# KirillKryukov/naf

Hardware: AMD Instinct MI355X
Metric: unnaf GB/s (uncompressed bases out) on 100 GB synthetic FASTA (higher is better)
Workload: dtype u8; 1 GPU; unnaf decode of a 100.0 GB synthetic-ACGT FASTA archive on one GPU (the size BASELINE.json's metric is quoted on; configs[1] at 10 GB rides along as cfg10_*), 100 records, 80-col lines; archive made in-run by the GPU ennaf; .naf 24739662224 B -> FASTA 99999995684 B, text + archive + decoded text resident in HBM; parallelism=one archive, one GPU, no data-path collective

## Files before the change

naf_amd/csrc/emit.hip:

```cpp
#include "ctx.h"
#include "wgscan.h"
#include "emit_core.h"
#include "packed.h"
#include <thread>

__device__ __forceinline__ void st_text16(u8 *p, const uint4 &v, int nt)
{
    if (nt) {
        u32x4 nv; nv.x = v.x; nv.y = v.y; nv.z = v.z; nv.w = v.w;
        __builtin_nontemporal_store(nv, (u32x4 *)p);
    } else *(uint4 *)p = v;
}

__global__ void k_len_flags(const u32 *units, u64 n, u64 *flag)
{
    u64 i = (u64)blockIdx.x * blockDim.x + threadIdx.x;
    if (i < n) flag[i] = units[i] != 0xFFFFFFFFu;
}
__global__ void k_len_acc(const u32 *units, u64 n, const u64 *ridx, u64 *rec_len, u64 N)
{
    u64 i = (u64)blockIdx.x * blockDim.x + threadIdx.x;
    if (i < n && ridx[i] < N) atomicAdd((unsigned long long *)&rec_len[ridx[i]], (unsigned long long)units[i]);
}

// ... 109 lines not shown
            if (v != 255) {
                if ((u64)nt + size > cap) { ok = false; break; }
                for (u32 k = t; k < size; k += 256) toggles[nt + k] = base + (u64)v * (k + 1);
                nt += size;
            }
            base += (u64)v * size; units += size; pos += 4;
        } else if (type == 0) {
            if ((u64)pos + 3 + size > len) { ok = false; break; }
            const u8 *rb = mbuf + pos + 3;
            const u32 per = (size + 255) / 256, lo = t * per < size ? t * per : size, hi = lo + per < size ? lo + per : size;
            u64 sm = 0, cn = 0;
            for (u32 k = lo; k < hi; k++) { const u32 u = rb[k]; sm += u; cn += u != 255; }
            u64 tot_s, tot_c;
            const u64 is = wg_scan_inclusive<u64, OpAdd>(sm, &tot_s, lds);
            const u64 ic = wg_scan_inclusive<u64, OpAdd>(cn, &tot_c, lds);
            if (nt + tot_c > cap) { ok = false; break; }
            u64 at = base + is - sm; u32 idx = nt + (u32)(ic - cn);
            for (u32 k = lo; k < hi; k++) { const u32 u = rb[k]; at += u; if (u != 255) toggles[idx++] = at; }
            base += tot_s; nt += (u32)tot_c; units += size; pos += 3 + size;
        } else ok = false;
        if (last) done = true;
    }
    ok = ok && done && pos == len && units == expect_units;
    if (t == 0) { res[0] = ok ? 1 : 0; res[1] = nt; res[2] = units; }
}

__device__ __forceinline__ void rec_size_of(u64 r, u64 len, const u64 *idz, const u64 *nmz, int has_ids, int has_names, int mode, u64 L, u32 *hdr, u64 *out)
{
    u64 h = 0;
    if (mode == EM_FASTA || mode == EM_FASTQ) {
        u64 idl = 0, nml = 0;
        if (has_ids) idl = idz[r] - (r ? idz[r - 1] + 1 : 0);
        if (has_names) nml = nmz[r] - (r ? nmz[r - 1] + 1 : 0);
        u64 name = has_ids ? idl + ((has_names && nml) ? 1 + nml : 0) : nml;
        h = 1 + name + 1;
    }
    u64 body;
    if (mode == EM_FASTQ) body = 2 * len + 4;
    else if (mode == EM_SEQUENCES) body = len + 1;
    else body = len ? len + (L ? (len + L - 1) / L : 1) : 0;
    *hdr = (u32)h; *out = h + body;
}
__global__ void k_rec_sizes(u64 N, const u64 *rec_len, const u64 *idz, const u64 *nmz, int has_ids, int has_names,
                            int mode, u64 L, u32 *hdr_len, u64 *out_size, u64 *base_size)
{
    u64 r = (u64)blockIdx.x * blockDim.x + threadIdx.x;
    if (r >= N) return;
// ... 535 lines not shown
        }
        if (g == 0) { os[len] = '\n'; os[len + 1] = '+'; os[len + 2] = '\n'; os[2 * len + 3] = '\n'; }
        group_copy<ER_LANES>(os + len + 3, P.qual + base, len, g);
    }
    if (!in_lds) return;
    __syncthreads();
    u8 *dst = out + wbase; const u32 n = (u32)wspan;
    u32 head = (u32)((16 - ((uintptr_t)dst & 15)) & 15); if (head > n) head = n;
    if (threadIdx.x < head) dst[threadIdx.x] = stage[threadIdx.x];
    u32 words = (n - head) >> 4;
    for (u32 w = threadIdx.x; w < words; w += WGT) {
        u64 a, b2; __builtin_memcpy(&a, stage + head + 16 * w, 8); __builtin_memcpy(&b2, stage + head + 16 * w + 8, 8);
        uint4 v; v.x = (u32)a; v.y = (u32)(a >> 32); v.z = (u32)b2; v.w = (u32)(b2 >> 32);
        st_text16(dst + head + 16 * w, v, P.nt_store);
    }
    for (u32 k = head + 16 * words + threadIdx.x; k < n; k += WGT) dst[k] = stage[k];
}

#define EMIT_TOG_LDS 256u
struct TileIdx { u64 gline, k, khi; u32 col, fast; };
#define TI_HDR 0xFFFFFFFFu
struct TileFlat { u64 q0, A, q1, A1, q2, qf; };
struct TileFlatE { u64 base, a1_addr; u32 a1_sh, K0, K1, d1, d2, qoff, par0, pad; };
static_assert(sizeof(TileFlatE) == sizeof(TileFlat), "the derived record replaces the raw one in place");
#define FLAT_QM 4096
#define TILE_WG 255
__global__ __launch_bounds__(256) void k_tile_index(EmitP P, u64 ntiles, TileIdx *ti, u64 *tr, u32 *list, u32 *count, TileFlat *tsig, u32 spare, u32 *list2)
{
    __shared__ u64 s_k[256], s_r[256];
    const u64 t = (u64)blockIdx.x * TILE_WG + threadIdx.x;
    const u64 p = P.out_begin + t * 4096;
    TileIdx x; x.fast = 0; x.gline = 0; x.khi = 0; x.k = P.n_toggles; x.col = TI_HDR;
    TileFlat f; f.q0 = f.A = f.q1 = f.A1 = f.q2 = f.qf = 0;
    u64 r = ~0ull; u32 cbits = 1;
    const bool inside = t < ntiles && p < P.out_end;
    if (inside) {
        u64 g;
        if (P.mode == EM_SEQ) { r = 0; x.col = 0; g = p; x.gline = p; }
        else {
            r = upper_bound_u64(P.rec_out, 0, P.N + 1, p) - 1;
            u64 off = p - P.rec_out[r], hl = P.hdr_len[r], len = P.rec_len[r], j = 0;
            if (off >= hl) {
                u64 q = off - hl;
                if (P.mode == EM_FASTA && P.L) {
                    u64 line = q / (P.L + 1), col = q - line * (P.L + 1);
                    j = line * P.L + (col < P.L ? col : P.L);
                    if (P.L < 0xFFFFFFF0ull) { x.gline = P.rec_base[r] + line * P.L; x.col = (u32)col; }
                } else if (P.mode != EM_FASTQ) { j = q; x.col = 0; x.gline = P.rec_base[r] + q; }
                if (j > len) j = len;
            }
            g = P.rec_base[r] + j;
        }
        x.k = P.masking ? upper_bound_u64(P.toggles, 0, P.n_toggles, g) : 0;
// ... 2 lines not shown
            const u64 q = g >> 1;
            u64 lo, hi, gs = q >> 13; if (gs >= P.fslots) gs = P.fslots - 1;
            if (si[gs].q0 <= q) { lo = gs; hi = gs + 1; u64 st = 1; while (hi < P.fslots && si[hi].q0 <= q) { lo = hi; st <<= 1; hi = lo + st; } if (hi > P.fslots) hi = P.fslots; }
            else { hi = gs; u64 st = 1; lo = gs - 1; while (lo > 0 && si[lo].q0 > q) { hi = lo; st <<= 1; lo = lo > st ? lo - st : 0; } }
            while (hi - lo > 1) { const u64 mid = (lo + hi) >> 1; if (si[mid].q0 <= q) lo = mid; else hi = mid; }
            f.q0 = si[lo].q0; f.A = si[lo].A; f.qf = q;
            if (P.fcls) {
                u32 c = 3; u64 b = lo >> 2; const u64 nb = P.fslots >> 2, qe = q + 2048 + 16;
                for (u32 k = 0; k < 6 && b < nb && si[4 * b].q0 <= qe; k++, b++) c &= P.fcls[b];
                if (b < nb && si[4 * b].q0 <= qe) c = 0;
                cbits = c;
            }
            u64 cs = lo + 1;
            while (cs < P.fslots && si[cs + 1].q0 == si[cs].q0) cs++;
            f.q1 = si[cs].q0; f.A1 = cs < P.fslots ? si[cs].A : 0;
            u64 ce = cs < P.fslots ? cs + 1 : cs;
            while (ce < P.fslots && si[ce + 1].q0 == si[ce].q0) ce++;
            f.q2 = si[ce].q0;
        }
    }
    s_k[threadIdx.x] = x.k; s_r[threadIdx.x] = r;
    __syncthreads();
    if (threadIdx.x == TILE_WG) return;
    TileFlatE e; e.base = (u64)P.fsrc; e.a1_addr = (u64)P.fsrc; e.a1_sh = 4; e.K0 = e.K1 = 0; e.d1 = e.d2 = 0x7FFFFFFFu; e.qoff = 0; e.par0 = 0; e.pad = 0;
    if (t >= ntiles) {
        if (t == ntiles) { tr[t] = ~0ull; ti[t] = x; if (tsig && spare) *(TileFlatE *)&tsig[t] = e; }
        else if (tsig && t < ntiles + spare) { ti[t].fast = 0; *(TileFlatE *)&tsig[t] = e; }
        return;
    }
    tr[t] = r;
    if (!inside) { ti[t] = x; if (tsig) *(TileFlatE *)&tsig[t] = e; list[atomicAdd(count, 1u)] = (u32)t; return; }
    const u64 r_next = s_r[threadIdx.x + 1];
    x.khi = s_k[threadIdx.x + 1];
    const bool wrap = P.mode == EM_FASTA && P.L != 0;
    bool fast = x.col != TI_HDR && r == r_next && P.out_begin + (t + 1) * 4096 <= P.out_end && !P.force_slow && (!wrap || P.L >= 16);
    bool packed = false;
    if (tsig) {
        packed = fast && (cbits & 2);
        if (fast && !(cbits & 1)) fast = false;
        if (fast) {
            fast = f.qf + 2048 + 16 < f.q2 || f.q2 == f.q1;
            if (P.ftail && f.qf + 2048 + 16 >= P.ftail_q) fast = false;
            if (f.q2 != f.q1 && (f.A1 > f.A ? f.A1 - f.A : f.A - f.A1) >= (1ull << 29)) fast = false;
        }
        if (fast) {
            const u64 gline = x.gline;
            const u64 dd1 = f.q1 - f.qf, dd2 = f.q2 - f.qf;
            e.d1 = dd1 > 0x7FFFFFFFull ? 0x7FFFFFFFu : (u32)dd1; e.d2 = dd2 > 0x7FFFFFFFull ? 0x7FFFFFFFu : (u32)dd2;
            const u64 T0 = f.A - 4 * (f.qf - f.q0), T1 = f.A1 + 4 * (u64)e.d1;
            const bool two = f.q2 != f.q1;
            const u64 tmin = two && T1 < T0 ? T1 : T0;
            const u64 ub = (tmin - 40 - 4 * (u64)FLAT_QM) & ~7ull;
            e.base = (u64)P.fsrc + (u64)((i64)ub >> 3);
            e.K0 = (u32)(T0 - 40 - ub); e.K1 = two ? (u32)(T1 - 40 - ub) : e.K0;
            e.qoff = (u32)((gline >> 1) - f.qf); e.par0 = (u32)gline & 1u;
            const u64 t1 = (f.A1 < 40 ? 40 : f.A1) - 40;
            e.a1_addr = (u64)P.fsrc + (t1 >> 3); e.a1_sh = (u32)(t1 & 7) + 4;
        }
        *(TileFlatE *)&tsig[t] = e;
    }
    x.fast = fast ? 1u : (packed ? 2u : 0u);
    ti[t] = x;
    if (!fast) { if (packed) list2[atomicAdd(count + 1, 1u)] = (u32)t; else list[atomicAdd(count, 1u)] = (u32)t; }
}

template <bool FOURBIT>
__device__ __forceinline__ void emit_tile_body(const EmitP &P, const TileIdx &a, u8 *out_tile)
{
    __shared__ u64 s_tog[EMIT_TOG_LDS];
    const u32 ntog = (u32)(a.khi - a.k < EMIT_TOG_LDS ? a.khi - a.k : EMIT_TOG_LDS);
    const bool use_tog = P.masking && a.k < a.khi && a.khi - a.k <= EMIT_TOG_LDS;
    if (use_tog) { for (u32 i = threadIdx.x; i < ntog; i += 256) s_tog[i] = P.toggles[a.k + i]; __syncthreads(); }
    const u32 lane16 = threadIdx.x * 16;
    u64 g0; u32 nl_b = 64;
    if (P.mode == EM_FASTA && P.L != 0) {
        const u32 Lp1 = (u32)P.L + 1;
        u32 c = a.col + lane16, dl;
        if (Lp1 < 32768) dl = __umulhi(c, P.Ldiv_magic); else dl = c >= Lp1 ? 1u : 0u;
        u32 col = c - dl * Lp1;
        g0 = a.gline + (u64)dl * (u32)P.L + col;
        u32 d = (u32)P.L - col;
        nl_b = d < 16 ? d : 64;
    } else g0 = a.gline + lane16;
    u64 lo, hi;
    if (FOURBIT) {
// ... 228 lines not shown
            u32 w0 = s_pair[h >> 24], w1 = s_pair[(h >> 16) & 0xFFu], w2 = s_pair[(h >> 8) & 0xFFu], w3 = s_pair[h & 0xFFu];
            if (g0 & 1) {
                const u32 c9 = s_pair[n9 << 4];
                w0 = __builtin_amdgcn_alignbyte(w1, w0, 1); w1 = __builtin_amdgcn_alignbyte(w2, w1, 1);
                w2 = __builtin_amdgcn_alignbyte(w3, w2, 1); w3 = __builtin_amdgcn_alignbyte(c9, w3, 1);
            }
            lo = (u64)w0 | ((u64)w1 << 32); hi = (u64)w2 | ((u64)w3 << 32);
        }
        const u32 ntog = (u32)(a.khi - a.k < EMIT_TOG_LDS ? a.khi - a.k : EMIT_TOG_LDS);
        const bool use_tog = P.masking && a.k < a.khi && a.khi - a.k <= EMIT_TOG_LDS;
        if (use_tog) mask16_from(s_tog[j], ntog, a.k, g0, lo, hi);
        else mask16(P, a.k, a.khi, P.masking && a.k < a.khi, g0, lo, hi);
        uint4 v; v.x = (u32)lo; v.y = (u32)(lo >> 32); v.z = (u32)hi; v.w = (u32)(hi >> 32);
        if (nls[j] < 16) {
            const uint4 sel = s_spl[2 * nls[j]], orv = s_spl[2 * nls[j] + 1];
            const u32 x0 = v.x, x1 = v.y, x2 = v.z, x3 = v.w;
            v.x = __builtin_amdgcn_perm(x0, 0u, sel.x) | orv.x; v.y = __builtin_amdgcn_perm(x1, x0, sel.y) | orv.y;
            v.z = __builtin_amdgcn_perm(x2, x1, sel.z) | orv.z; v.w = __builtin_amdgcn_perm(x3, x2, sel.w) | orv.w;
        }
        st_text16(out + t * 4096 + lane16, v, P.nt_store);
    }
}

template <u32 TW>
__global__ __launch_bounds__(64) void k_emit_tile_flat_wave(EmitP P, const TileIdx *ti, const TileFlat *tsig, u8 *out, u64 ntiles, u32 xcd_chunk)
{
    u32 wg = blockIdx.x;
    if (xcd_chunk) { wg = (blockIdx.x & 7u) * xcd_chunk + (blockIdx.x >> 3); if ((u64)wg * TW >= ntiles) return; }
    __shared__ u64 s_tog[TW][EMIT_TOG_LDS];
    __shared__ uint4 s_spl[32];
    __shared__ u32 s_pair[256];
    const u32 lane = threadIdx.x;
    if (lane < 32) s_spl[lane] = ((const uint4 *)(P.fpair + 272))[lane];
    ((uint4 *)s_pair)[lane] = ((const uint4 *)(P.fpair + 16))[lane];
    TileIdx A[TW]; TileFlatE F[TW]; bool live[TW];
    {
        const u64 t0 = (u64)wg * TW;
        const uint4 *pa = (const uint4 *)(ti + t0), *pf = (const uint4 *)(tsig + t0);
        uint4 ra[2 * TW], rf[3 * TW];
#pragma unroll
        for (u32 i = 0; i < 2 * TW; i++) ra[i] = pa[i];
#pragma unroll
        for (u32 i = 0; i < 3 * TW; i++) rf[i] = pf[i];
#pragma unroll
        for (u32 j = 0; j < TW; j++) {
            __builtin_memcpy(&A[j], &ra[2 * j], 32); __builtin_memcpy(&F[j], &rf[3 * j], 48);
            live[j] = t0 + j < ntiles && A[j].fast == 1;
        }
    }
    u64 X[TW][4]; u32 grels[TW][4], pk[TW][4];
#pragma unroll
    for (u32 j = 0; j < TW; j++) {
        const TileIdx &a = A[j]; const TileFlatE &e = F[j];
#pragma unroll
        for (u32 r = 0; r < 4; r++) {
            const u32 lane16 = (r * 64 + lane) * 16;
            u32 grel, nl_b = 64;
            if (P.mode == EM_FASTA && P.L != 0) {
                const u32 Lp1 = (u32)P.L + 1;
                u32 c = a.col + lane16, dl;
                if (Lp1 < 32768) dl = __umulhi(c, P.Ldiv_magic); else dl = c >= Lp1 ? 1u : 0u;
                u32 col = c - dl * Lp1;
                grel = dl * (u32)P.L + col;
                u32 d = (u32)P.L - col;
                nl_b = d < 16 ? d : 64;
            } else grel = lane16;
            grels[j][r] = grel;
            const u32 par = e.par0 + grel;
            const u32 need = 8 + (par & 1u);
            const u32 qrel = (par >> 1) + e.qoff;
            const bool second = qrel >= e.d1;
            const u32 qm = live[j] ? ~0u : 0u;
            const u32 off = (second ? e.K1 : e.K0) - ((4 * qrel) & qm);
            const u32 rem = (second ? e.d2 : e.d1) - qrel;
            X[j][r] = ldg_at_unaligned<u64>(e.base + (off >> 3));
            pk[j][r] = nl_b | ((need > rem ? rem : 16u) << 8) | ((off & 7u) << 16);
        }
    }
    if (P.masking) {
#pragma unroll
        for (u32 j = 0; j < TW; j++) {
            const u64 nt = A[j].khi - A[j].k;
            for (u32 i = lane; i < EMIT_TOG_LDS; i += 64) s_tog[j][i] = (live[j] && i < nt && nt <= EMIT_TOG_LDS) ? P.toggles[A[j].k + i] : 0ull;
        }
    }
    __syncthreads();
#pragma unroll
    for (u32 j = 0; j < TW; j++) {
        const u64 t = (u64)wg * TW + j;
        if (!live[j]) continue;
        const TileIdx &a = A[j];
        const u32 ntog = (u32)(a.khi - a.k < EMIT_TOG_LDS ? a.khi - a.k : EMIT_TOG_LDS);
        const bool use_tog = P.masking && a.k < a.khi && a.khi - a.k <= EMIT_TOG_LDS;
#pragma unroll
        for (u32 r = 0; r < 4; r++) {
            const u64 g0 = a.gline + grels[j][r];
            const u32 nl = pk[j][r] & 0xFFu, have = (pk[j][r] >> 8) & 0xFFu;
            u64 h36 = X[j][r] >> ((pk[j][r] >> 16) + 4);
            if (have < 9) {
                const u64 y = ldg_at_unaligned<u64>(F[j].a1_addr);
                const u64 n36 = (y >> F[j].a1_sh) & 0xFFFFFFFFFull;
                const u32 keep = 4 * have;
                h36 = (h36 & ~(0xFFFFFFFFFull >> keep)) | (n36 >> keep);
            }
            const u32 h = (u32)(h36 >> 4), n9 = (u32)h36 & 15u;
            u64 lo, hi;
            {
                u32 w0 = s_pair[h >> 24], w1 = s_pair[(h >> 16) & 0xFFu], w2 = s_pair[(h >> 8) & 0xFFu], w3 = s_pair[h & 0xFFu];
                if (g0 & 1) {
                    const u32 c9 = s_pair[n9 << 4];
                    w0 = __builtin_amdgcn_alignbyte(w1, w0, 1); w1 = __builtin_amdgcn_alignbyte(w2, w1, 1);
                    w2 = __builtin_amdgcn_alignbyte(w3, w2, 1); w3 = __builtin_amdgcn_alignbyte(c9, w3, 1);
                }
                lo = (u64)w0 | ((u64)w1 << 32); hi = (u64)w2 | ((u64)w3 << 32);
            }
            if (use_tog) mask16_from(s_tog[j], ntog, a.k, g0, lo, hi);
            else mask16(P, a.k, a.khi, P.masking && a.k < a.khi, g0, lo, hi);
            uint4 v; v.x = (u32)lo; v.y = (u32)(lo >> 32); v.z = (u32)hi; v.w = (u32)(hi >> 32);
            if (nl < 16) {
                const uint4 sel = s_spl[2 * nl], orv = s_spl[2 * nl + 1];
                const u32 x0 = v.x, x1 = v.y, x2 = v.z, x3 = v.w;
                v.x = __builtin_amdgcn_perm(x0, 0u, sel.x) | orv.x; v.y = __builtin_amdgcn_perm(x1, x0, sel.y) | orv.y;
                v.z = __builtin_amdgcn_perm(x2, x1, sel.z) | orv.z; v.w = __builtin_amdgcn_perm(x3, x2, sel.w) | orv.w;
            }
            st_text16(out + t * 4096 + (r * 64 + lane) * 16, v, P.nt_store);
        }
    }
}

template <bool FOURBIT>
__device__ __forceinline__ void emit_rest_tile(const EmitP &P, const TileIdx *ti, const u64 *tr, u64 t, u8 *out, u32 chunk)
{
    const TileIdx a = ti[t];
    u64 p0 = P.out_begin + t * 4096 + chunk * 16;
    if (p0 >= P.out_end) return;
    u32 nbytes = P.out_end - p0 < 16 ? (u32)(P.out_end - p0) : 16;
    const u32 Lp1_32 = (P.L + 1) >> 32 ? 0 : (u32)(P.L + 1);
    u8 *o = out + (p0 - P.out_begin);
    if (P.mode == EM_SEQ) {
        for (u32 bb = 0; bb < nbytes; bb++) o[bb] = (u8)emit_byte<FOURBIT>(P, p0 + bb, 0, 0, a.k, a.khi);
// ... 169 lines not shown
{
    ContainerOut *d_co = arena_new<ContainerOut>(c, 1); if (!d_co) return NAF_GPU_ENOMEM;
    LAUNCH(c, "unnaf_parse_container", k_parse_container, 1, 64, 0, (const u8 *)d_naf, (u64)len, d_co);
    int rc = ctx_readback(c, co, d_co, sizeof *co); if (rc) return rc;
    if (co->code) { char buf[160]; container_error_text(co->code, &co->h, buf, sizeof buf); return ctx_fail(c, NAF_GPU_EFORMAT, "%s", buf); }
    return 0;
}

extern "C" int naf_gpu_parse_header(naf_gpu_ctx *c, const void *d_naf, size_t len, naf_gpu_header *h)
{
    if (!c || !h) return NAF_GPU_EARG;
    arena_reset(c);
    ContainerOut co;
    int rc = parse_container_device(c, d_naf, len, &co);
    *h = co.h;
    return rc;
}

enum { S_IDS = 0, S_NAMES, S_LEN, S_MASK, S_SEQ, S_QUAL };

struct UnnafPlan {
    naf_gpu_header h; u8 frame_head[6][24]; EmitP P; u64 total; bool fourbit; bool empty;
    u64 seq_bytes; bool need_qual;
    u64 main_total, surplus, sur_c, sur_base0;
};

static int load_section(naf_gpu_ctx *c, const u8 *d_naf, const naf_gpu_header &h, int i, u64 expect, const char *what, u8 **out, const u8 *head = nullptr)
{
    u8 *buf = (u8 *)arena_alloc(c, expect + 32);
    if (!buf) return NAF_GPU_ENOMEM;
    size_t n = 0;
    int rc = zstd_decode(c, d_naf + h.payload_off[i], h.comp_size[i], 0, buf, expect, &n, head);
    if (rc == NAF_GPU_ECAP || (rc == 0 && n != expect)) return ctx_fail(c, NAF_GPU_EFORMAT, "can't decompress %s\n", what);
    if (rc) return rc;
    *out = buf;
    return 0;
}

static int unnaf_prepare(naf_gpu_ctx *c, const u8 *d_naf, size_t naf_len, const naf_gpu_unnaf_opts *o, UnnafPlan &pl)
{
    ContainerOut co;
    int rc = parse_container_device(c, d_naf, naf_len, &co); if (rc) return rc;
    pl.h = co.h; memcpy(pl.frame_head, co.frame_head, sizeof pl.frame_head);
    const naf_gpu_header &h = pl.h;
    EmitP &P = pl.P; memset(&P, 0, sizeof P);
    int has_mask = (h.flags >> 2) & 1, has_data = (h.flags >> 1) & 1, has_qual = h.flags & 1;
// ... 93 lines not shown
    HIP_TRY(x, hipMemsetAsync(rec_len, 0, (N + 1) * 8, x->stream));
    if (n_len) LAUNCH(x, "unnaf_len_flags", k_len_flags, cdiv(n_len, 256), 256, 0, (const u32 *)lens, n_len, flag);
    if ((r = scan_exclusive_u64(x, flag, n_len, flag + n_len + 1))) return r;
    if (n_len) LAUNCH(x, "unnaf_len_acc", k_len_acc, cdiv(n_len, 256), 256, 0, (const u32 *)lens, n_len, (const u64 *)flag, rec_len, N);
    u64 nrec = 0;
    if ((r = ctx_readback(x, &nrec, flag + n_len + 1, 8))) return r;
    if (nrec < N) return ctx_fail(x, NAF_GPU_EFORMAT, "corrupted lengths: %llu records described, %llu expected", (unsigned long long)nrec, (unsigned long long)N);
    return 0;
}

static int mask_rle_frame(naf_gpu_ctx *x, SideCall &S, bool *done)
{
    const naf_gpu_header &h = S.h; EmitP &P = S.P;
    const u64 cs = h.comp_size[S_MASK], n_mask = h.orig_size[S_MASK];
    *done = false;
    if (!(cs >= 4 && cs <= MASK_RLE_SRC && n_mask >= 2 * cs) || ctx_opt_is(x, "MASK_RLE", '0')) return 0;
    const u8 fhd = S.pl.frame_head[S_MASK][0];
    const u32 fcs_flag = fhd >> 6, single = (fhd >> 5) & 1;
    const u32 hdr_size = 1 + (single ? 0 : 1) + (fcs_flag == 0 ? single : (fcs_flag == 1 ? 2 : (fcs_flag == 2 ? 4 : 8)));
    if ((fhd & 0x0F) || hdr_size >= cs) return 0;
    u64 *tg = arena_new<u64>(x, MASK_RLE_TOG + 1), *d_res = arena_new<u64>(x, 4);
    if (!tg || !d_res) return NAF_GPU_ENOMEM;
    LAUNCH(x, "unnaf_mask_rle", k_mask_rle_frame, 1, 256, (u32)((cs + 15) & ~15ull), S.d_naf + h.payload_off[S_MASK], (u32)cs, hdr_size, n_mask, tg, MASK_RLE_TOG, d_res);
    u64 res[3] = { 0, 0, 0 };
    int r = ctx_readback(x, res, d_res, 24); if (r) return r;
    if (res[0] == 1) { P.toggles = tg; P.n_toggles = res[1]; *done = true; }
    return 0;
}

static int mask_toggles(naf_gpu_ctx *x, SideCall &S)
{
    const naf_gpu_header &h = S.h; EmitP &P = S.P;
    int r; bool done;
    u8 *mu = nullptr; const u64 n_mask = h.orig_size[S_MASK];
    if ((r = mask_rle_frame(x, S, &done)) || done) return r;
    if ((r = load_section(x, S.d_naf, h, S_MASK, n_mask, "mask", &mu, S.pl.frame_head[S_MASK]))) return r;
    u64 tiles = (n_mask + MT_TILE - 1) / MT_TILE;
    u64 *ts = arena_new<u64>(x, tiles + 2), *tc = arena_new<u64>(x, tiles + 2);
    if (!ts || !tc) return NAF_GPU_ENOMEM;
    if (tiles) LAUNCH(x, "unnaf_mask_count", k_mask_count, tiles, 256, 0, (const u8 *)mu, n_mask, ts, tc);
    if ((r = scan_exclusive_u64(x, ts, tiles, (u64 *)nullptr))) return r;
    if ((r = scan_exclusive_u64(x, tc, tiles, tc + tiles + 1))) return r;
    u64 ntog = 0;
    if ((r = ctx_readback(x, &ntog, tc + tiles + 1, 8))) return r;
    u64 *tg = arena_new<u64>(x, ntog + 1);
    if (!tg) return NAF_GPU_ENOMEM;
    if (tiles) LAUNCH(x, "unnaf_mask_scatter", k_mask_scatter, tiles, 256, 0, (const u8 *)mu, n_mask, (const u64 *)ts, (const u64 *)tc, tg, ntog);
    P.toggles = tg; P.n_toggles = ntog;
    return 0;
}

static void side_mask_meanwhile(naf_gpu_ctx *c, SideCall &S)
{
    if (!S.mask_meanwhile) return;
    S.mask_ran = true; S.rc_mask = mask_toggles(c, S);
    if (S.rc_mask) memcpy(S.mask_err, c->err, sizeof c->err);
}

static int side_fused_launch(naf_gpu_ctx *x, SideCall &S, u64 st[6], bool *done)
{
    const naf_gpu_header &h = S.h; EmitP &P = S.P;
    const u64 N = h.n_sequences;
    SectionJobs j; u8 *buf[3] = { nullptr, nullptr, nullptr };
    int r = section_jobs(x, S, j); if (r) return r;
    SideJob J; memset(&J, 0, sizeof J);
    for (int q = 0; q < j.m; q++) { J.cap[q] = (u32)j.cap[q]; J.len[q] = (u32)j.len[q]; buf[j.k[q]] = j.dst[q]; }
    u32 *d_res = nullptr;
    if ((r = zstd_small_launch(x, j.m, j.src, j.len, j.dst, j.cap, &d_res))) return r;
    J.res = d_res; J.n_jobs = (u32)j.m;
    J.ids = buf[0]; J.ids_n = h.orig_size[S_IDS]; J.names = buf[1]; J.names_n = h.orig_size[S_NAMES];
    J.lens = (const u32 *)buf[2]; J.n_len = h.orig_size[S_LEN] / 4;
// ... 143 lines not shown
    S.mask_meanwhile = P.masking && !mask_beside && P.mode != EM_SEQ && aux;
    CtxJoinGuard mask_joined{ mask_beside ? aux_mask : nullptr };
    if (mask_beside) ctx_worker_start(aux_mask, [&] { S.rc_mask = mask_toggles(aux_mask, S); });
    int rc = unnaf_sections_main(c, S, aux, aux_names);
    const hipError_t mask_synced = mask_beside ? ctx_side_join(aux_mask) : hipSuccess;
    if (rc) return rc;
    if (mask_beside) { if (S.rc_mask) { ctx_take_error(c, aux_mask); return S.rc_mask; } SIDE_SYNC_TRY(c, mask_synced, aux_mask); return 0; }
    if (S.mask_ran) { if (S.rc_mask) ctx_take_error(c, S.mask_err); return S.rc_mask; }
    return P.masking ? mask_toggles(c, S) : 0;
}

#include "payload.h"

struct UnnafCall {
    naf_gpu_ctx *c; const u8 *d_naf;
    UnnafPlan pl;
    ZSplit split; ZFlat zflat;
    bool whole, size_only; u64 out_begin, out_end; u8 *d_out; size_t out_cap, *out_len;
    bool ranged = false; u64 s_lo = 0, s_hi = 0, q_lo = 0, q_hi = 0;
    u64 rec0 = 0, rec1 = 0;
    bool has_main = false, has_tail = false;
    bool payload_done = false;
    bool fuse_on, flat_fuse, emit_wave; const char *emit; int split_parts;
    bool try_flat = false;
    UnnafCall() { split.parts = 0; split.done = 0; split.status = nullptr; memset(&zflat, 0, sizeof zflat); }
    ~UnnafCall() { zstd_flat_drop(&zflat); }
};

static void unnaf_switches(UnnafCall &U)
{
    const naf_gpu_ctx *c = U.c;
    U.fuse_on = ctx_opt_is(c, "FUSE", '1');
    U.flat_fuse = !ctx_opt_is(c, "FLAT_FUSE", '0');
    U.emit = ctx_opt(c, "EMIT");
    U.emit_wave = !ctx_opt_is(c, "EMIT_WAVE", '0');
    const char *nsp = ctx_opt(c, "SPLIT");
    U.split_parts = nsp ? atoi(nsp) : 4;
}

static int payload_seq(UnnafCall &U)
{
    PayloadSpan sp;
    int r = payload_range(U.c, U.d_naf, U.pl, S_SEQ, U.s_lo, U.s_hi, U.ranged ? PAYLOAD_RANGE : PAYLOAD_WHOLE, &sp);
    if (!r) U.pl.P.seq = sp.base;
    return r;
}
static int payload_qual(UnnafCall &U, naf_gpu_ctx *qc)
{
    PayloadSpan sp;
    int r = payload_range(qc, U.d_naf, U.pl, S_QUAL, U.q_lo, U.q_hi, U.ranged ? PAYLOAD_RANGE : PAYLOAD_WHOLE, &sp);
    if (!r) U.pl.P.qual = sp.base;
    return r;
}

static int unnaf_fork_sides(UnnafCall &U)
{
    naf_gpu_ctx *c = U.c; UnnafPlan &pl = U.pl; const u8 *d_naf = U.d_naf;
    arena_reset(c->side);
    HIP_TRY(c, hipEventRecord(c->fork_ev, c->stream));
    HIP_TRY(c, hipStreamWaitEvent(c->side->stream, c->fork_ev, 0));
// ... 126 lines not shown
    if (pl.P.mode == EM_FASTA || pl.P.mode == EM_FASTQ) {
        u64 nr = rec1 - rec0 + 1, htot = 0;
        u64 *ho = arena_new<u64>(c, nr + 2); if (!ho) return NAF_GPU_ENOMEM;
        LAUNCH(c, "unnaf_hdr_len64", k_hdr_len64, cdiv(nr, 256), 256, 0, pl.P.hdr_len, rec0, nr, ho);
        if ((rc = scan_exclusive_u64(c, ho, nr, ho + nr + 1))) return rc;
        if ((rc = ctx_readback(c, &htot, ho + nr + 1, 8))) return rc;
        u8 *ht = (u8 *)arena_alloc(c, htot + 32); if (!ht) return NAF_GPU_ENOMEM;
        LAUNCH(c, "unnaf_hdr_build", k_hdr_build, cdiv(nr, 32), 256, 0, pl.P, rec0, nr, (const u64 *)ho, ht);
        pl.P.hdr_off = ho; pl.P.hdr_text = ht; pl.P.hdr_r0 = rec0;
    }
    u32 grid = cdiv(pl.P.out_end - pl.P.out_begin, ES_SPAN);
    LAUNCH_4BIT(pl.fourbit, c, "unnaf_emit_short", k_emit_short, grid, 256, pl.P, d_out);
    return 0;
}

static int emit_span(UnnafCall &U)
{
    naf_gpu_ctx *c = U.c; UnnafPlan &pl = U.pl; u8 *d_out = U.d_out;
    u32 grid = cdiv(pl.P.out_end - pl.P.out_begin, EMIT_SPAN);
    LAUNCH_4BIT(pl.fourbit, c, "unnaf_emit", k_emit, grid, 256, pl.P, d_out);
    return 0;
}

struct TileCall { u64 ntiles; TileIdx *ti; u64 *tr; u32 *list, *list2, *cnt; TileFlat *tsig; naf_gpu_ctx *ic, *xc; u64 t_done; };

static void launch_tiles(UnnafCall &U, const TileCall &T, naf_gpu_ctx *x, u64 t0, u64 t1)
{
    const UnnafPlan &pl = U.pl; u8 *d_out = U.d_out; const TileIdx *ti = T.ti;
    if (U.emit_wave && pl.fourbit) LAUNCH(x, "unnaf_emit", (k_emit_tile_wave<true, 2>), cdiv(t1 - t0, 2u), 64, 0, pl.P, (const TileIdx *)(ti + t0), d_out + t0 * 4096, (u64)(t1 - t0));
    else if (U.emit_wave) LAUNCH(x, "unnaf_emit", (k_emit_tile_wave<false, 2>), cdiv(t1 - t0, 2u), 64, 0, pl.P, (const TileIdx *)(ti + t0), d_out + t0 * 4096, (u64)(t1 - t0));
    else LAUNCH_4BIT(pl.fourbit, x, "unnaf_emit", k_emit_tile, (u32)(t1 - t0), 256, pl.P, (const TileIdx *)(ti + t0), d_out + t0 * 4096);
}

static int tile_index(UnnafCall &U, TileCall &T)
{
    naf_gpu_ctx *c = U.c; UnnafPlan &pl = U.pl; const ZFlat &zflat = U.zflat;
    const u64 ntiles = T.ntiles = cdiv(pl.P.out_end - pl.P.out_begin, 4096);
    TileIdx *ti = T.ti = arena_new<TileIdx>(c, ntiles + 2 + FLAT_TPW); u64 *tr = T.tr = arena_new<u64>(c, ntiles + 2);
    u32 *list = T.list = arena_new<u32>(c, ntiles + 1), *cnt = T.cnt = arena_new<u32>(c, 2);
    u32 *list2 = T.list2 = (zflat.ready && zflat.cls) ? arena_new<u32>(c, ntiles + 1) : list;
    if (!ti || !tr || !list || !cnt || !list2) return NAF_GPU_ENOMEM;
    u64 Lp1 = pl.P.L + 1;
    pl.P.Ldiv_magic = (Lp1 >= 2 && Lp1 < 32768) ? (u32)((1ull << 32) / Lp1 + 1) : 0;
    naf_gpu_ctx *ic = T.ic = U.split.done ? c->side2 : c;
    HIP_TRY(c, hipMemsetAsync(cnt, 0, 8, ic->stream));
    TileFlat *tsig = T.tsig = nullptr;
    if (zflat.ready) {
        tsig = T.tsig = arena_new<TileFlat>(c, ntiles + 2 + FLAT_TPW); u32 *fpair = arena_new<u32>(c, 400); if (!tsig || !fpair) return NAF_GPU_ENOMEM;
        LAUNCH(ic, "unnaf_flat_pair", k_flat_pair, 1, 256, 0, pl.P, fpair);
        pl.P.fpair = fpair;
    }
    LAUNCH(ic, "unnaf_tile_index", k_tile_index, cdiv(ntiles + 1 + FLAT_TPW, TILE_WG), 256, 0, pl.P, ntiles, ti, tr, list, cnt, tsig, (u32)FLAT_TPW, list2);
    T.xc = c; T.t_done = 0;
    if (zflat.ready && zflat.aux) {
        HIP_TRY(c, hipEventRecord(c->split_ev[0], c->stream));
        if (!zflat.later) { HIP_TRY(c, hipStreamWaitEvent(zflat.aux->stream, c->split_ev[0], 0)); T.xc = zflat.aux; }
    }
    return 0;
}

static int tiles_behind_split_parts(UnnafCall &U, TileCall &T)
{
    naf_gpu_ctx *c = U.c, *ic = T.ic; const UnnafPlan &pl = U.pl; const ZSplit &split = U.split;
    HIP_TRY(c, hipEventRecord(c->split_ev[ZSPLIT_MAX], ic->stream));
    for (int k = 0; k + 1 < split.parts; k++) {
        u64 bases_ready = split.out_end[k] * (pl.fourbit ? 2u : 1u);
        u64 t_hi = bases_ready / 4096; t_hi = t_hi > 1 ? t_hi - 1 : 0;
        if (t_hi > T.ntiles) t_hi = T.ntiles;
        if (t_hi <= T.t_done) continue;
        HIP_TRY(c, hipStreamWaitEvent(ic->stream, split.ev[k], 0));
        launch_tiles(U, T, ic, T.t_done, t_hi);
        T.t_done = t_hi;
    }
    HIP_TRY(c, hipEventRecord(c->split_ev[ZSPLIT_MAX + 1], ic->stream));
    HIP_TRY(c, hipStreamWaitEvent(c->stream, c->split_ev[ZSPLIT_MAX], 0));
    return 0;
}

static int flat_tiles(UnnafCall &U, TileCall &T)
{
    naf_gpu_ctx *c = U.c; UnnafPlan &pl = U.pl; ZFlat &zflat = U.zflat; u8 *d_out = U.d_out;
    const u64 ntiles = T.ntiles; const TileIdx *ti = T.ti; const TileFlat *tsig = T.tsig;
    int rc;
    const bool flat_job = zflat.later != nullptr;
    const u32 nwg = cdiv(ntiles, 4u), chunk = (nwg + 7) / 8;
    const bool mixed = flat_job || (zflat.cls && zflat.n_decoded);
    const bool wave = U.emit_wave && (!mixed || zflat.n_walk == 0);
    if (wave && pl.P.masking && pl.P.n_toggles >= ntiles) { const u32 ch = ((u32)ntiles + 7) / 8; LAUNCH(c, "unnaf_emit_flat", k_emit_tile_flat_wave<1>, ch * 8, 64, 0, pl.P, (const TileIdx *)ti, (const TileFlat *)tsig, d_out, (u64)ntiles, ch); }
    else if (wave) { const u32 ch = (cdiv(ntiles, 2u) + 7) / 8; LAUNCH(c, "unnaf_emit_flat", k_emit_tile_flat_wave<2>, ch * 8, 64, 0, pl.P, (const TileIdx *)ti, (const TileFlat *)tsig, d_out, (u64)ntiles, ch); }
    else LAUNCH(c, "unnaf_emit_flat", k_emit_tile_flat<4>, chunk * 8, 256, 0, pl.P, (const TileIdx *)ti, (const TileFlat *)tsig, d_out, (u64)ntiles, chunk);
    if (flat_job) {
        if ((rc = zstd_flat_later(c, &zflat))) return rc;
        if (zflat.aux) T.xc = zflat.aux;
    }
    if (zflat.cls && zflat.n_decoded) {
        const u64 est = (u64)zflat.n_decoded * 64 + 64;
        const u32 lgrid = (u32)(est < ntiles ? (est < 16384 ? est : 16384) : (ntiles < 16384 ? ntiles : 16384));
        naf_gpu_ctx *xc = T.xc; const u32 *list2 = T.list2, *cnt = T.cnt;
        if (wave) LAUNCH(xc, "unnaf_emit", k_emit_tile_list_wave<true>, lgrid, 64, 0, pl.P, (const TileIdx *)ti, (const u32 *)list2, (const u32 *)(cnt + 1), d_out);
        else LAUNCH(xc, "unnaf_emit", k_emit_tile_list<true>, lgrid, 256, 0, pl.P, (const TileIdx *)ti, (const u32 *)list2, (const u32 *)(cnt + 1), d_out);
    }
    return 0;
}

static void rest_tiles(UnnafCall &U, const TileCall &T)
{
    const UnnafPlan &pl = U.pl; u8 *d_out = U.d_out; naf_gpu_ctx *xc = T.xc;
    const u64 ntiles = T.ntiles; const TileIdx *ti = T.ti; const u64 *tr = T.tr; const u32 *list = T.list, *cnt = T.cnt;
    const u32 rest_grid = 4u * (u32)(ntiles < EMIT_REST_GRID ? ntiles : EMIT_REST_GRID);
    LAUNCH_4BIT(pl.fourbit, xc, "unnaf_emit_rest", k_emit_rest, rest_grid, 64, pl.P, (const TileIdx *)ti, (const u64 *)tr, (const u32 *)list, (const u32 *)cnt, d_out);
}

static int emit_tiles(UnnafCall &U)
{
    naf_gpu_ctx *c = U.c; TileCall T;
    int rc = tile_index(U, T); if (rc) return rc;
    if (U.split.done && (rc = tiles_behind_split_parts(U, T))) return rc;
    if (U.zflat.ready) { if ((rc = flat_tiles(U, T))) return rc; }
    else if (T.t_done < T.ntiles) launch_tiles(U, T, c, T.t_done, T.ntiles);
    rest_tiles(U, T);
    if (T.xc != c) { HIP_TRY(c, hipEventRecord(c->split_ev[1], T.xc->stream)); HIP_TRY(c, hipStreamWaitEvent(c->stream, c->split_ev[1], 0)); }
    if (U.split.done) HIP_TRY(c, hipStreamWaitEvent(c->stream, c->split_ev[ZSPLIT_MAX + 1], 0));
    if (U.zflat.ready && ctx_tracing(c)) {
        u32 hc[2] = { 0, 0 };
        if (!ctx_readback(c, hc, T.cnt, 8)) ctx_trace(c, "[flat tiles] total %llu rest %u decoded %u\n", (unsigned long long)T.ntiles, hc[0], hc[1]);
    }
    return 0;
}

static int emit_records(UnnafCall &U)
{
    const UnnafPlan &pl = U.pl;
    const char *ek = U.emit;
    bool short_rec = pl.P.mode != EM_SEQ && pl.total / pl.P.N < 16384;
    if (ek && !strcmp(ek, "short")) short_rec = pl.P.mode != EM_SEQ;
    if (ek && !strcmp(ek, "long")) short_rec = false;
    if (pl.P.force_slow) { short_rec = false; ek = "span"; }
    if (U.whole && pl.P.mode == EM_FASTQ && !pl.P.force_slow && !(ek && ek[0])) return emit_fastq_records(U);
    if (short_rec) return emit_short_records(U);
    if (ek && !strcmp(ek, "span")) return emit_span(U);
    return emit_tiles(U);
}

static void emit_surplus(UnnafCall &U)
{
    naf_gpu_ctx *c = U.c; const UnnafPlan &pl = U.pl;
    const u64 lo = (U.out_begin > pl.main_total ? U.out_begin : pl.main_total) - pl.main_total, hi = U.out_end - pl.main_total;
    u8 *dst = U.d_out + (pl.main_total + lo - U.out_begin);
// ... 104 lines not shown
```

Measured before the change: 4250 GB/s.

## Add unmasked flat emit path and split tile indexing across streams

Detects archives with no lowercase mask (zero toggles, or one toggle past the sequence end) and, when so, runs a specialised flat-wave emit kernel. That kernel skips TileIdx loads, toggle staging in LDS and masking, and reads the column and fast flag packed into the TileFlatE record. Fast tiles also stop writing TileIdx. Tile indexing is split into a small first slice on the main stream and the rest on the aux stream, so emit of the first slice can start while the remainder is still indexed. This adds event synchronisation and an extra readback of the single toggle. The LDS size argument tied to FLAT_WAVES8 is meant to change occupancy.

```diff
diff --git a/naf_amd/csrc/emit.hip b/naf_amd/csrc/emit.hip
--- a/naf_amd/csrc/emit.hip
+++ b/naf_amd/csrc/emit.hip
@@ -155,7 +155,8 @@
         if (last) done = true;
     }
     ok = ok && done && pos == len && units == expect_units;
-    if (t == 0) { res[0] = ok ? 1 : 0; res[1] = nt; res[2] = units; }
+    __syncthreads();
+    if (t == 0) { res[0] = ok ? 1 : 0; res[1] = nt; res[2] = units; res[3] = nt == 0 ? ~0ull : (nt == 1 ? toggles[0] : 0); }
 }
 
 __device__ __forceinline__ void rec_size_of(u64 r, u64 len, const u64 *idz, const u64 *nmz, int has_ids, int has_names, int mode, u64 L, u32 *hdr, u64 *out)
@@ -737,13 +738,18 @@
 #define TI_HDR 0xFFFFFFFFu
 struct TileFlat { u64 q0, A, q1, A1, q2, qf; };
 struct TileFlatE { u64 base, a1_addr; u32 a1_sh, K0, K1, d1, d2, qoff, par0, pad; };
+#define TFE_FAST 0x80000000u
 static_assert(sizeof(TileFlatE) == sizeof(TileFlat), "the derived record replaces the raw one in place");
 #define FLAT_QM 4096
 #define TILE_WG 255
-__global__ __launch_bounds__(256) void k_tile_index(EmitP P, u64 ntiles, TileIdx *ti, u64 *tr, u32 *list, u32 *count, TileFlat *tsig, u32 spare, u32 *list2)
+#define TIDX_LAST 1u
+#define TIDX_FLAT_OWN 2u
+#define TIDX_SKIP_FAST 4u
+__global__ __launch_bounds__(256) void k_tile_index(EmitP P, u64 ntiles, TileIdx *ti, u64 *tr, u32 *list, u32 *count, TileFlat *tsig, u32 spare, u32 *list2,
+                                                    u64 t_first, u64 t_end, u32 how)
 {
     __shared__ u64 s_k[256], s_r[256];
-    const u64 t = (u64)blockIdx.x * TILE_WG + threadIdx.x;
+    const u64 t = t_first + (u64)blockIdx.x * TILE_WG + threadIdx.x;
     const u64 p = P.out_begin + t * 4096;
     TileIdx x; x.fast = 0; x.gline = 0; x.khi = 0; x.k = P.n_toggles; x.col = TI_HDR;
     TileFlat f; f.q0 = f.A = f.q1 = f.A1 = f.q2 = f.qf = 0;
@@ -792,6 +798,7 @@
     s_k[threadIdx.x] = x.k; s_r[threadIdx.x] = r;
     __syncthreads();
     if (threadIdx.x == TILE_WG) return;
+    if (t >= t_end && !((how & TIDX_LAST) && t >= ntiles)) return;
     TileFlatE e; e.base = (u64)P.fsrc; e.a1_addr = (u64)P.fsrc; e.a1_sh = 4; e.K0 = e.K1 = 0; e.d1 = e.d2 = 0x7FFFFFFFu; e.qoff = 0; e.par0 = 0; e.pad = 0;
     if (t >= ntiles) {
         if (t == ntiles) { tr[t] = ~0ull; ti[t] = x; if (tsig && spare) *(TileFlatE *)&tsig[t] = e; }
@@ -827,10 +834,11 @@
             const u64 t1 = (f.A1 < 40 ? 40 : f.A1) - 40;
             e.a1_addr = (u64)P.fsrc + (t1 >> 3); e.a1_sh = (u32)(t1 & 7) + 4;
         }
+        if (how & TIDX_FLAT_OWN) { e.pad = x.col; if (fast) e.a1_sh |= TFE_FAST; }
         *(TileFlatE *)&tsig[t] = e;
     }
     x.fast = fast ? 1u : (packed ? 2u : 0u);
-    ti[t] = x;
+    if (!(fast && (how & TIDX_SKIP_FAST))) ti[t] = x;
     if (!fast) { if (packed) list2[atomicAdd(count + 1, 1u)] = (u32)t; else list[atomicAdd(count, 1u)] = (u32)t; }
 }
 
@@ -1105,12 +1113,12 @@
     }
 }
 
-template <u32 TW>
+template <u32 TW, bool MASKED = true>
 __global__ __launch_bounds__(64) void k_emit_tile_flat_wave(EmitP P, const TileIdx *ti, const TileFlat *tsig, u8 *out, u64 ntiles, u32 xcd_chunk)
 {
     u32 wg = blockIdx.x;
     if (xcd_chunk) { wg = (blockIdx.x & 7u) * xcd_chunk + (blockIdx.x >> 3); if ((u64)wg * TW >= ntiles) return; }
-    __shared__ u64 s_tog[TW][EMIT_TOG_LDS];
+    __shared__ u64 s_tog[MASKED ? TW : 1][MASKED ? EMIT_TOG_LDS : 1];
     __shared__ uint4 s_spl[32];
     __shared__ u32 s_pair[256];
     const u32 lane = threadIdx.x;
@@ -1121,17 +1129,24 @@
         const u64 t0 = (u64)wg * TW;
         const uint4 *pa = (const uint4 *)(ti + t0), *pf = (const uint4 *)(tsig + t0);
         uint4 ra[2 * TW], rf[3 * TW];
-#pragma unroll
-        for (u32 i = 0; i < 2 * TW; i++) ra[i] = pa[i];
+        if (MASKED) {
+#pragma unroll
+            for (u32 i = 0; i < 2 * TW; i++) ra[i] = pa[i];
+        }
 #pragma unroll
         for (u32 i = 0; i < 3 * TW; i++) rf[i] = pf[i];
 #pragma unroll
         for (u32 j = 0; j < TW; j++) {
-            __builtin_memcpy(&A[j], &ra[2 * j], 32); __builtin_memcpy(&F[j], &rf[3 * j], 48);
-            live[j] = t0 + j < ntiles && A[j].fast == 1;
-        }
-    }
-    u64 X[TW][4]; u32 grels[TW][4], pk[TW][4];
+            __builtin_memcpy(&F[j], &rf[3 * j], 48);
+            if (MASKED) { __builtin_memcpy(&A[j], &ra[2 * j], 32); live[j] = t0 + j < ntiles && A[j].fast == 1; }
+            else {
+                A[j].gline = 0; A[j].k = A[j].khi = 0; A[j].col = F[j].pad; A[j].fast = 0;
+                live[j] = t0 + j < ntiles && (F[j].a1_sh & TFE_FAST) != 0;
+                F[j].a1_sh &= ~TFE_FAST;
+            }
+        }
+    }
+    u64 X[TW][4]; u32 grels[MASKED ? TW : 1][4], pk[TW][4];
 #pragma unroll
     for (u32 j = 0; j < TW; j++) {
         const TileIdx &a = A[j]; const TileFlatE &e = F[j];
@@ -1148,7 +1163,7 @@
                 u32 d = (u32)P.L - col;
                 nl_b = d < 16 ? d : 64;
             } else grel = lane16;
-            grels[j][r] = grel;
+            if (MASKED) grels[j][r] = grel;
             const u32 par = e.par0 + grel;
             const u32 need = 8 + (par & 1u);
             const u32 qrel = (par >> 1) + e.qoff;
@@ -1157,14 +1172,14 @@
             const u32 off = (second ? e.K1 : e.K0) - ((4 * qrel) & qm);
             const u32 rem = (second ? e.d2 : e.d1) - qrel;
             X[j][r] = ldg_at_unaligned<u64>(e.base + (off >> 3));
-            pk[j][r] = nl_b | ((need > rem ? rem : 16u) << 8) | ((off & 7u) << 16);
-        }
-    }
-    if (P.masking) {
+            pk[j][r] = nl_b | ((need > rem ? rem : 16u) << 8) | ((off & 7u) << 16) | (MASKED ? 0u : (par & 1u) << 24);
+        }
+    }
+    if (MASKED && P.masking) {
 #pragma unroll
         for (u32 j = 0; j < TW; j++) {
             const u64 nt = A[j].khi - A[j].k;
-            for (u32 i = lane; i < EMIT_TOG_LDS; i += 64) s_tog[j][i] = (live[j] && i < nt && nt <= EMIT_TOG_LDS) ? P.toggles[A[j].k + i] : 0ull;
+            for (u32 i = lane; i < EMIT_TOG_LDS; i += 64) s_tog[MASKED ? j : 0][MASKED ? i : 0] = (live[j] && i < nt && nt <= EMIT_TOG_LDS) ? P.toggles[A[j].k + i] : 0ull;
         }
     }
     __syncthreads();
@@ -1174,12 +1189,12 @@
         if (!live[j]) continue;
         const TileIdx &a = A[j];
         const u32 ntog = (u32)(a.khi - a.k < EMIT_TOG_LDS ? a.khi - a.k : EMIT_TOG_LDS);
-        const bool use_tog = P.masking && a.k < a.khi && a.khi - a.k <= EMIT_TOG_LDS;
+        const bool use_tog = MASKED && P.masking && a.k < a.khi && a.khi - a.k <= EMIT_TOG_LDS;
 #pragma unroll
         for (u32 r = 0; r < 4; r++) {
-            const u64 g0 = a.gline + grels[j][r];
+            const u64 g0 = MASKED ? a.gline + grels[MASKED ? j : 0][r] : (u64)(pk[j][r] >> 24);
             const u32 nl = pk[j][r] & 0xFFu, have = (pk[j][r] >> 8) & 0xFFu;
-            u64 h36 = X[j][r] >> ((pk[j][r] >> 16) + 4);
+            u64 h36 = X[j][r] >> (((pk[j][r] >> 16) & 7u) + 4);
             if (have < 9) {
                 const u64 y = ldg_at_unaligned<u64>(F[j].a1_addr);
                 const u64 n36 = (y >> F[j].a1_sh) & 0xFFFFFFFFFull;
@@ -1197,8 +1212,10 @@
                 }
                 lo = (u64)w0 | ((u64)w1 << 32); hi = (u64)w2 | ((u64)w3 << 32);
             }
-            if (use_tog) mask16_from(s_tog[j], ntog, a.k, g0, lo, hi);
-            else mask16(P, a.k, a.khi, P.masking && a.k < a.khi, g0, lo, hi);
+            if (MASKED) {
+                if (use_tog) mask16_from(s_tog[MASKED ? j : 0], ntog, a.k, g0, lo, hi);
+                else mask16(P, a.k, a.khi, P.masking && a.k < a.khi, g0, lo, hi);
+            }
             uint4 v; v.x = (u32)lo; v.y = (u32)(lo >> 32); v.z = (u32)hi; v.w = (u32)(hi >> 32);
             if (nl < 16) {
                 const uint4 sel = s_spl[2 * nl], orv = s_spl[2 * nl + 1];
@@ -1414,6 +1431,7 @@
 struct UnnafPlan {
     naf_gpu_header h; u8 frame_head[6][24]; EmitP P; u64 total; bool fourbit; bool empty;
     u64 seq_bytes; bool need_qual;
+    bool no_lower = false;
     u64 main_total, surplus, sur_c, sur_base0;
 };
 
@@ -1553,9 +1571,9 @@
     u64 *tg = arena_new<u64>(x, MASK_RLE_TOG + 1), *d_res = arena_new<u64>(x, 4);
     if (!tg || !d_res) return NAF_GPU_ENOMEM;
     LAUNCH(x, "unnaf_mask_rle", k_mask_rle_frame, 1, 256, (u32)((cs + 15) & ~15ull), S.d_naf + h.payload_off[S_MASK], (u32)cs, hdr_size, n_mask, tg, MASK_RLE_TOG, d_res);
-    u64 res[3] = { 0, 0, 0 };
-    int r = ctx_readback(x, res, d_res, 24); if (r) return r;
-    if (res[0] == 1) { P.toggles = tg; P.n_toggles = res[1]; *done = true; }
+    u64 res[4] = { 0, 0, 0, 0 };
+    int r = ctx_readback(x, res, d_res, 32); if (r) return r;
+    if (res[0] == 1) { P.toggles = tg; P.n_toggles = res[1]; S.pl.no_lower = res[3] >= h.orig_size[S_SEQ];       *done = true; }
     return 0;
 }
 
@@ -1578,6 +1596,9 @@
     if (!tg) return NAF_GPU_ENOMEM;
     if (tiles) LAUNCH(x, "unnaf_mask_scatter", k_mask_scatter, tiles, 256, 0, (const u8 *)mu, n_mask, (const u64 *)ts, (const u64 *)tc, tg, ntog);
     P.toggles = tg; P.n_toggles = ntog;
+    u64 first = ~0ull;
+    if (ntog == 1 && (r = ctx_readback(x, &first, tg, 8))) return r;
+    S.pl.no_lower = ntog <= 1 && first >= h.orig_size[S_SEQ];
     return 0;
 }
 
@@ -1767,6 +1788,7 @@
     bool has_main = false, has_tail = false;
     bool payload_done = false;
     bool fuse_on, flat_fuse, emit_wave; const char *emit; int split_parts;
+    bool flat_unmasked, flat_waves8, flat_skip_ti; long long index_cut;
     bool try_flat = false;
     UnnafCall() { split.parts = 0; split.done = 0; split.status = nullptr; memset(&zflat, 0, sizeof zflat); }
     ~UnnafCall() { zstd_flat_drop(&zflat); }
@@ -1781,6 +1803,11 @@
     U.emit_wave = !ctx_opt_is(c, "EMIT_WAVE", '0');
     const char *nsp = ctx_opt(c, "SPLIT");
     U.split_parts = nsp ? atoi(nsp) : 4;
+    U.flat_unmasked = !ctx_opt_is(c, "FLAT_UNMASKED", '0');
+    U.flat_waves8 = !ctx_opt_is(c, "FLAT_WAVES8", '0');
+    U.flat_skip_ti = !ctx_opt_is(c, "FLAT_SKIP_TI", '0');
+    const char *cut = ctx_opt(c, "INDEX_CUT");
+    U.index_cut = cut && cut[0] ? atoll(cut) : -1;
 }
 
 static int payload_seq(UnnafCall &U)
@@ -1953,7 +1980,23 @@
     return 0;
 }
 
-struct TileCall { u64 ntiles; TileIdx *ti; u64 *tr; u32 *list, *list2, *cnt; TileFlat *tsig; naf_gpu_ctx *ic, *xc; u64 t_done; };
+struct TileCall { u64 ntiles; TileIdx *ti; u64 *tr; u32 *list, *list2, *cnt; TileFlat *tsig; naf_gpu_ctx *ic, *xc; u64 t_done; bool own; u64 cut; };
+
+static bool flat_emit_by_wave(const UnnafCall &U)
+{
+    const ZFlat &zflat = U.zflat;
+    const bool mixed = zflat.later != nullptr || (zflat.cls && zflat.n_decoded);
+    return U.emit_wave && (!mixed || zflat.n_walk == 0);
+}
+#define INDEX_CUT_MIN (1ull << 20)
+#define INDEX_CUT_SHARE 16
+static u64 index_cut(const UnnafCall &U, u64 ntiles)
+{
+    const ZFlat &zflat = U.zflat;
+    if (!zflat.ready || !zflat.aux || zflat.later || zflat.cls || U.split.done || U.index_cut == 0) return 0;
+    u64 cut = U.index_cut > 0 ? (u64)U.index_cut : (ntiles >= INDEX_CUT_MIN ? ntiles / INDEX_CUT_SHARE : 0);
+    return cut < ntiles ? cut & ~7ull : 0;
+}
 
 static void launch_tiles(UnnafCall &U, const TileCall &T, naf_gpu_ctx *x, u64 t0, u64 t1)
 {
@@ -1981,7 +2024,18 @@
         LAUNCH(ic, "unnaf_flat_pair", k_flat_pair, 1, 256, 0, pl.P, fpair);
         pl.P.fpair = fpair;
     }
-    LAUNCH(ic, "unnaf_tile_index", k_tile_index, cdiv(ntiles + 1 + FLAT_TPW, TILE_WG), 256, 0, pl.P, ntiles, ti, tr, list, cnt, tsig, (u32)FLAT_TPW, list2);
+    T.own = zflat.ready && U.flat_unmasked && (!pl.P.masking || pl.no_lower) && !U.split.done && flat_emit_by_wave(U);
+    const u32 how = T.own ? TIDX_FLAT_OWN | (U.flat_skip_ti ? TIDX_SKIP_FAST : 0u) : 0u;
+    const u64 cut = T.cut = index_cut(U, ntiles);
+    if (cut) {
+        naf_gpu_ctx *ax = zflat.aux;
+        HIP_TRY(c, hipEventRecord(c->split_ev[2], c->stream));
+        HIP_TRY(c, hipStreamWaitEvent(ax->stream, c->split_ev[2], 0));
+        LAUNCH(c, "unnaf_tile_index", k_tile_index, cdiv(cut, TILE_WG), 256, 0, pl.P, ntiles, ti, tr, list, cnt, tsig, (u32)FLAT_TPW, list2, (u64)0, cut, how);
+        LAUNCH(ax, "unnaf_tile_index", k_tile_index, cdiv(ntiles - cut + 1 + FLAT_TPW, TILE_WG), 256, 0, pl.P, ntiles, ti, tr, list, cnt, tsig, (u32)FLAT_TPW, list2, cut, ntiles, how | TIDX_LAST);
+        HIP_TRY(c, hipEventRecord(c->split_ev[3], ax->stream));
+    } else
+        LAUNCH(ic, "unnaf_tile_index", k_tile_index, cdiv(ntiles + 1 + FLAT_TPW, TILE_WG), 256, 0, pl.P, ntiles, ti, tr, list, cnt, tsig, (u32)FLAT_TPW, list2, (u64)0, ntiles, how | TIDX_LAST);
     T.xc = c; T.t_done = 0;
     if (zflat.ready && zflat.aux) {
         HIP_TRY(c, hipEventRecord(c->split_ev[0], c->stream));
@@ -2014,12 +2068,22 @@
     const u64 ntiles = T.ntiles; const TileIdx *ti = T.ti; const TileFlat *tsig = T.tsig;
     int rc;
     const bool flat_job = zflat.later != nullptr;
-    const u32 nwg = cdiv(ntiles, 4u), chunk = (nwg + 7) / 8;
-    const bool mixed = flat_job || (zflat.cls && zflat.n_decoded);
-    const bool wave = U.emit_wave && (!mixed || zflat.n_walk == 0);
-    if (wave && pl.P.masking && pl.P.n_toggles >= ntiles) { const u32 ch = ((u32)ntiles + 7) / 8; LAUNCH(c, "unnaf_emit_flat", k_emit_tile_flat_wave<1>, ch * 8, 64, 0, pl.P, (const TileIdx *)ti, (const TileFlat *)tsig, d_out, (u64)ntiles, ch); }
-    else if (wave) { const u32 ch = (cdiv(ntiles, 2u) + 7) / 8; LAUNCH(c, "unnaf_emit_flat", k_emit_tile_flat_wave<2>, ch * 8, 64, 0, pl.P, (const TileIdx *)ti, (const TileFlat *)tsig, d_out, (u64)ntiles, ch); }
-    else LAUNCH(c, "unnaf_emit_flat", k_emit_tile_flat<4>, chunk * 8, 256, 0, pl.P, (const TileIdx *)ti, (const TileFlat *)tsig, d_out, (u64)ntiles, chunk);
+    const bool wave = flat_emit_by_wave(U);
+    auto emit_range = [&](u64 t0, u64 t1) {
+        const u64 n = t1 - t0; const TileIdx *rti = ti + t0; const TileFlat *rts = tsig + t0; u8 *ro = d_out + t0 * 4096;
+        if (wave && pl.P.masking && !T.own && pl.P.n_toggles >= ntiles) { const u32 ch = (u32)((n + 7) / 8); LAUNCH(c, "unnaf_emit_flat", k_emit_tile_flat_wave<1>, ch * 8, 64, 0, pl.P, rti, rts, ro, n, ch); }
+        else if (wave && T.own) {
+            const u32 ch = (u32)(((n + 1) / 2 + 7) / 8), lds = U.flat_waves8 ? 0u : 4096u;
+            LAUNCH(c, "unnaf_emit_flat", (k_emit_tile_flat_wave<2, false>), ch * 8, 64, lds, pl.P, rti, rts, ro, n, ch);
+        }
+        else if (wave) { const u32 ch = (u32)(((n + 1) / 2 + 7) / 8); LAUNCH(c, "unnaf_emit_flat", k_emit_tile_flat_wave<2>, ch * 8, 64, 0, pl.P, rti, rts, ro, n, ch); }
+        else { const u32 ch = (u32)(((n + 3) / 4 + 7) / 8); LAUNCH(c, "unnaf_emit_flat", k_emit_tile_flat<4>, ch * 8, 256, 0, pl.P, rti, rts, ro, n, ch); }
+    };
+    if (T.cut) {
+        emit_range(0, T.cut);
+        HIP_TRY(c, hipStreamWaitEvent(c->stream, c->split_ev[3], 0));
+        emit_range(T.cut, ntiles);
+    } else emit_range(0, ntiles);
     if (flat_job) {
         if ((rc = zstd_flat_later(c, &zflat))) return rc;
         if (zflat.aux) T.xc = zflat.aux;
@@ -2054,7 +2118,8 @@
     if (U.split.done) HIP_TRY(c, hipStreamWaitEvent(c->stream, c->split_ev[ZSPLIT_MAX + 1], 0));
     if (U.zflat.ready && ctx_tracing(c)) {
         u32 hc[2] = { 0, 0 };
-        if (!ctx_readback(c, hc, T.cnt, 8)) ctx_trace(c, "[flat tiles] total %llu rest %u decoded %u\n", (unsigned long long)T.ntiles, hc[0], hc[1]);
+        if (!ctx_readback(c, hc, T.cnt, 8)) ctx_trace(c, "[flat tiles] total %llu rest %u decoded %u unmasked %d cut %llu toggles %llu no_lower %d\n", (unsigned long long)T.ntiles, hc[0], hc[1], T.own ? 1 : 0, (unsigned long long)T.cut,
+                                                         (unsigned long long)U.pl.P.n_toggles, U.pl.no_lower ? 1 : 0);
     }
     return 0;
 }
```

After: 4240 GB/s. About the same (-0.2%).
